# Luca96/carla-driving-rl-agent

Hardware: AMD Instinct MI355X
Metric: PPO update-steps/sec (batch=256, 4x90x120x3 obs) (higher is better)
Workload: dtype f32; 1 GPU; configs[1]: synthetic rollout buffer 256x4-frame 90x120x3 obs per GPU, full CARLANetwork fwd/bwd + PPO (re-sampled Beta, pathwise) / value loss + clip + Adam, fp32; per_gpu_batch=256, global_batch=256, parallelism=dp1, policy_loss=resampled (reference-faithful)

## Files before the change

### carla-driving-rl-agent_amd/_lib.py

```python
import ctypes as C
import os

_HERE = os.path.dirname(os.path.abspath(__file__))
LIB_PATH = os.path.join(_HERE, 'libcdrl_hip.so')


class CdrlError(RuntimeError):
    pass


class Config(C.Structure):
    _fields_ = [('B', C.c_int32), ('T', C.c_int32), ('H', C.c_int32), ('W', C.c_int32),
                ('road', C.c_int32), ('vehicle', C.c_int32), ('navigation', C.c_int32), ('A', C.c_int32),
                ('stem', C.c_int32), ('stage_c', C.c_int32 * 3), ('stage_n', C.c_int32 * 3), ('last', C.c_int32),
                ('feat', C.c_int32), ('rnn_image', C.c_int32), ('rnn_small', C.c_int32), ('dyn', C.c_int32),
                ('head', C.c_int32), ('exp_scale', C.c_float), ('compute', C.c_int32),
                ('freeze_trunk', C.c_int32), ('optimizer', C.c_int32), ('polyak', C.c_float), ('train_stats', C.c_int32),
                ('clip_mode', C.c_int32), ('skip_nonfinite', C.c_int32)]


class TrainStatsLayout(C.Structure):
    _fields_ = [(n, C.c_int32) for n in ('rows', 'width', 'header', 'kind', 't_head', 't_dynamics', 'lr', 'lr_dynamics', 'clip_ratio',
                                         'entropy_coef', 'speed', 'similarity', 'metrics', 'norms', 'trunk_norms', 'n_policy',
                                         'n_value', 'n_trunk')]
# ... 54 lines not shown

_i, _i64, _f, _d, _sz = C.c_int, C.c_int64, C.c_float, C.c_double, C.c_size_t
_L = C.c_void_p
_V = C.POINTER(View)
_pp = C.POINTER(C.c_void_p)

PROTOTYPES = {
    'cdrl_last_error': (C.c_char_p, []),
    'cdrl_version': (_i, []),
    'cdrl_env_overrides': (_i, [C.c_char_p, _i]),
    'cdrl_diag_active': (_i, []),
    'cdrl_crc32c': (C.c_uint32, [C.c_uint32, C.c_void_p, C.c_size_t]),
    'cdrl_config_default': (None, [C.POINTER(Config)]),
    'cdrl_optimizer_slots': (_i, [_i, C.POINTER(C.c_int32), C.POINTER(C.c_float)]),
    'cdrl_learner_create': (_i, [C.POINTER(Config), C.POINTER(_L)]),
    'cdrl_learner_destroy': (None, [_L]),
    'cdrl_learner_param_count': (_i, [_L, _i]),
    'cdrl_learner_param_info': (_i, [_L, _i, _i, C.POINTER(ParamInfo)]),
    'cdrl_learner_region_offset': (_i64, [_L, _i, _i]),
    'cdrl_learner_region_elems': (_i64, [_L, _i, _i]),
    'cdrl_learner_params_total': (_i64, [_L]),
    'cdrl_learner_grads_total': (_i64, [_L]),
    'cdrl_learner_workspace_bytes': (_sz, [_L]),
    'cdrl_learner_bind': (_i, [_L, _fp, _fp, _fp, _fp, _fp, _sz]),
    'cdrl_learner_set_hparams': (_i, [_L, C.POINTER(HParams), _fp]),
    'cdrl_learner_share_hparams': (_i, [_L, _L]),
    'cdrl_learner_set_comm_stream': (_i, [_L, _fp]),
    'cdrl_learner_tail_offset': (_i64, [_L]),
    'cdrl_learner_reset_optimizer_steps': (_i, [_L, _fp]),
    'cdrl_learner_get_optimizer_state': (_i, [_L, C.POINTER(OptimizerState), _fp]),
    'cdrl_learner_set_optimizer_state': (_i, [_L, C.POINTER(OptimizerState), _fp]),
    'cdrl_learner_gate_stats': (_i, [_L, C.POINTER(GateStats), _fp]),
    'cdrl_learner_gate_reset': (_i, [_L, _fp]),
    'cdrl_learner_train_stats_layout': (_i, [_L, C.POINTER(TrainStatsLayout)]),
    'cdrl_learner_train_stats_buffer': (_i, [_L, C.POINTER(C.c_void_p), C.POINTER(_i64)]),
    'cdrl_learner_train_stats_reset': (_i, [_L, _fp]),
    'cdrl_learner_policy_forward_backward': (_i, [_L, C.POINTER(PolicyBatch), _f, _fp]),
    'cdrl_learner_policy_forward': (_i, [_L, _fp, _fp, _fp, _fp, _fp]),
    'cdrl_learner_policy_backward': (_i, [_L, C.POINTER(PolicyBatch), _f, _fp]),
    'cdrl_learner_policy_forward_backward_resample': (_i, [_L, C.POINTER(PolicyBatch), C.c_uint64, C.c_uint64, _f, _fp]),
    'cdrl_pwconv_x3_packed_bytes': (_i64, [_i]),
    'cdrl_pwconv_x3_packed_bytes_n': (_i64, [_i, _i]),
    'cdrl_pwconv_x3_partial_rows': (_i, [_i, _i, _i, _i]),
    'cdrl_pwconv_x3_pack': (_i, [_fp, _i, _i, _i, _i, _fp, _fp]),
    'cdrl_pwconv_x3': (_i, [_fp, _i, _i, _fp, _fp, _fp, _fp, _i, _i, _i, _i, _i, _i, _fp, _fp]),
    'cdrl_pwconv_x3_wide_bwd_rows': (_i, [_i]),
    'cdrl_pwconv_x3_wide_bwd': (_i, [_fp, _i, _i, _i, _i, _fp, _fp, _fp, _fp, _fp, _i, _i, _i, _i, _i, _i, _i, _fp, _fp, _fp, _fp, _fp]),
    'cdrl_pwconv_bwd_fused_workspace': (_i64, [_i, _i, _i, _i, _i]),
    'cdrl_pwconv_bwd_fused': (_i, [_fp, _i, _i, _i, _i, _fp, _fp, _fp, _fp, _i, _i, _fp, _fp, _fp, _fp, _fp, _fp, _fp, C.c_void_p, _fp, _i,
                                   _i, _i, _fp, _fp, _fp, C.c_void_p, _i, _i, _i, _i, C.c_void_p]),
    'cdrl_gemm_x3_packed_bytes': (_i64, [_i, _i]),
    'cdrl_gemm_x3_pack': (_i, [_fp, _i, _i, _i, _i, _fp, _fp]),
    'cdrl_gemm_x3': (_i, [_fp, _i, _i, _fp, _fp, _fp, _i, _i, _i, _i, _i, _i, _fp]),
    'cdrl_f32_to_bf16': (_i, [_fp, _fp, _i64, _fp]),
    'cdrl_bf16_to_f32': (_i, [_fp, _fp, _i64, _fp]),
    'cdrl_pwconv_bf16_partial_rows': (_i, [_i, _i, _i, _i]),
    'cdrl_pwconv_bf16_packed_elems': (_i64, [_i]),
    'cdrl_pwconv_bf16_pack': (_i, [_fp, _i, _i, _fp, _fp]),
    'cdrl_pwconv_bf16': (_i, [_fp, _i, _i, _fp, _fp, _fp, _fp, _fp, _i, _i, _i, _i, _i, _i, _fp, _fp]),
    'cdrl_gru_step_fwd': (_i, [_fp] * 9 + [_i, _i, _fp]),
    'cdrl_gru_step_bwd': (_i, [_fp, _i] + [_fp] * 9 + [_i, _i, _fp]),
    'cdrl_beta_sample_logp': (_i, [_fp, _fp, _i, _i, _i, C.c_uint64, C.c_uint64, _fp, _fp, _fp]),
    'cdrl_beta_sample': (_i, [_fp, _fp, _i, _i, _i, C.c_uint64, C.c_uint64, _fp, _fp, _fp, _fp]),
    'cdrl_beta_act': (_i, [_fp, _fp, _i, _i, _i, C.c_uint64, C.c_uint64, _fp, _fp, _fp, _fp, _fp]),
    'cdrl_gamma_implicit_grad': (_i, [_fp, _fp, _i, _fp, _fp]),
    'cdrl_beta_sample_gammas': (_i, [_fp, _fp, _i, _i, _i, C.c_uint64, C.c_uint64, _fp, _fp]),
    'cdrl_philox_words': (_i, [C.c_uint64, C.c_uint64, C.c_uint64, _i, _i, _fp, _fp]),
    'cdrl_learner_policy_apply': (_i, [_L, _fp]),
    'cdrl_learner_joint_forward_backward': (_i, [_L, C.POINTER(PolicyBatch), _fp, _f, _fp]),
    'cdrl_learner_joint_forward_backward_resample': (_i, [_L, C.POINTER(PolicyBatch), _fp, C.c_uint64, C.c_uint64, _f, _fp]),
    'cdrl_learner_joint_apply': (_i, [_L, _fp]),
    'cdrl_learner_clone_forward_backward': (_i, [_L, C.POINTER(CloneBatch), _f, _f, _f, _f, _fp]),
    'cdrl_learner_repr_forward_backward': (_i, [_L, _fp, _fp, _fp, _fp, _f, _f, _fp]),
    'cdrl_learner_trunk_apply': (_i, [_L, _fp]),
    'cdrl_learner_sequence_begin': (_i, [_L, _fp]),
    'cdrl_learner_sequence_end': (_i, [_L, _fp]),
    'cdrl_learner_value_forward_backward': (_i, [_L, C.POINTER(ValueBatch), _f, _fp]),
    'cdrl_learner_value_apply': (_i, [_L, _fp]),
    'cdrl_learner_update_old_policy': (_i, [_L, _fp]),
    'cdrl_learner_predict': (_i, [_L, _fp, _fp, _fp, _fp, _fp, _fp, _fp, _fp]),
    'cdrl_learner_trunk_forward_train': (_i, [_L, _fp, _fp, _fp, _fp, _fp]),
    'cdrl_learner_get_buffer': (_i, [_L, _i, C.POINTER(_fp), C.POINTER(_i64)]),
    'cdrl_learner_named_buffer': (_i, [_L, C.c_char_p, C.POINTER(C.c_void_p), C.POINTER(_i64)]),
    'cdrl_learner_check_guards': (_i, [_L, _fp, C.POINTER(_i64), C.POINTER(_i64)]),
    'cdrl_gae_returns': (_i, [_fp, _fp, _i, _d, _d, _f, _fp, _fp, _fp, _fp, _fp, _fp]),
    'cdrl_gae_returns_segments': (_i, [_fp, _fp, _fp, _i, _i, _d, _d, _f, _fp, _fp, _fp, _fp, _fp, _fp]),
    'cdrl_gae_segments_scratch_doubles': (_i64, [_i, _i]),
    'cdrl_gather_rows': (_i, [_fp, _fp, _fp, _i, _i64, _fp]),
    'cdrl_gemm_nn': (_i, [_fp, _i, _i, _fp, _i, _i, _fp, _fp, _i, _i, _i, _i, _i, _i, _fp]),
    'cdrl_gemm_tn_workspace_elems': (_i64, [_i, _i, _i]),
    'cdrl_gemm_tn': (_i, [_fp, _i, _i, _fp, _i, _i, _fp, _i, _i, _i, _fp, _i, _fp]),
    'cdrl_bn_small_fwd': (_i, [_fp, _i, _i, _fp, _fp, _fp, _fp, _fp, _fp, _fp]),
    'cdrl_bn_small_bwd': (_i, [_fp, _fp, _i, _i, _fp, _fp, _fp, _fp, _fp, _fp]),
    'cdrl_bn_small_bwd_pair': (_i, [_fp, _fp, _fp, _i, _i] + [_fp] * 10),
    'cdrl_linear_heads_fwd': (_i, [_fp, _i, _fp, _fp, _fp, _fp, _i, _i, _fp]),
    'cdrl_linear_heads_bwd': (_i, [_fp, _i, _fp, _fp, _fp, _fp, _fp, _fp, _i, _i, _fp]),
    'cdrl_stem_fwd': (_i, [_fp, _fp, _fp, _fp, _i, _i, _i, _i, _i, _fp]),
    'cdrl_stem_fwd_stats_rows': (_i, [_i] * 5),
    'cdrl_stem_fwd_stats': (_i, [_fp] * 5 + [_i] * 5 + [_fp]),
    'cdrl_stem_bwd_workspace_doubles': (_i64, [_i, _i, _i, _i, _i]),
    'cdrl_stem_bwd_filter': (_i, [_fp, _fp, _fp, _fp, _i, _i, _i, _i, _i, _fp, _fp]),
    'cdrl_dwconv_fwd': (_i, [_fp, _fp, _fp, _fp, _i, _i, _i, _i, _i, _fp]),
    'cdrl_dwconv_bwd_data': (_i, [_fp, _fp, _fp, _i, _i, _i, _i, _i, _fp]),
    'cdrl_dwconv_bwd_workspace_doubles': (_i64, [_i, _i, _i, _i, _i]),
    'cdrl_dwconv_bwd_filter': (_i, [_fp, _fp, _fp, _fp, _i, _i, _i, _i, _i, _fp, _fp]),
    'cdrl_augment_workspace_floats': (_i64, [_i, _i, _i]),
# ... 122 lines not shown
```

### carla-driving-rl-agent_amd/csrc/capi.hip

```cpp
#include <stdlib.h>
#include <string.h>

#include <new>

#include "../../include/cdrl.h"
#include "engine.h"

using namespace cdrl;

struct cdrl_learner {
    Learner* impl;
};

static inline hipStream_t S(void* s) { return reinterpret_cast<hipStream_t>(s); }

#define CHECK_L(l)                         \
    if (!(l) || !(l)->impl) {              \
        cdrl::set_error("null learner");   \
        return -1;                         \
    }

static inline bool bad_act_type(int at) {
    if (at == 0 || at == 1) return false;
    cdrl::set_error("act_type: 0 (float32) or 1 (bf16)");
// ... 718 lines not shown
    }
    PwBwdFused f;
    f.dz = make_view(const_cast<float*>(dz), ld_dz, dz_coff);
    f.dz_shuffle = dz_shuffle;
    f.act = act;
    f.y = y;
    f.stats = stats;
    f.coef = coef;
    f.a = make_view(const_cast<float*>(a), lda, a_coff);
    f.a_stats = a_stats;
    f.a_gamma = a_gamma;
    f.a_beta = a_beta;
    f.a_dgamma = a_dgamma;
    f.a_dbeta = a_dbeta;
    f.a_coef = a_coef;
    f.W = W;
    f.Wp = W_packed;
    f.da = make_view(da, ldda, da_coff);
    f.accumulate = accumulate;
    f.dW = dW;
    f.db = db;
    f.qpart = qpart;
    f.dbpart = dbpart;
    f.G = G;
    f.Mg = Mg;
    f.N = N;
    f.K = K;
    f.at = act_type;
    CDRL_TRY(pw_bwd_fused(f, S(stream)));
    return pw_bwd_fused_reduce(f, S(stream));
}

int64_t cdrl_gemm_x3_packed_bytes(int N, int K) { return gemm_x3_packed_bytes(N, K); }

int cdrl_gemm_x3_pack(const float* B, int K, int N, int sbk, int sbn, void* packed, void* stream) {
    if (!B || !packed) return -1;
    GemmX3Pack e = gemm_x3_pack_entry(B, packed, K, N, sbk, sbn);
    GemmX3Pack* d = nullptr;
    if (hipMalloc(reinterpret_cast<void**>(&d), sizeof(e)) != hipSuccess) return -2;
    int rc = hipMemcpy(d, &e, sizeof(e), hipMemcpyHostToDevice) == hipSuccess ? gemm_x3_pack_many(d, 1, S(stream)) : -2;
    (void)hipStreamSynchronize(S(stream));
    (void)hipFree(d);
    return rc;
}

int cdrl_gemm_x3(const float* A, int lda, int a_coff, const void* B_packed, const float* bias, float* C, int ldc, int c_coff, int M,
                 int N, int K, int accumulate, int act_type, void* stream) {
    if (!A || !B_packed || !C) {
        cdrl::set_error("cdrl_gemm_x3: null argument");
        return -1;
    }
    return gemm_x3(make_view(const_cast<float*>(A), lda, a_coff), B_packed, bias, make_view(C, ldc, c_coff), M, N, K, accumulate,
                   S(stream), act_type != 0, act_type);
}

int cdrl_f32_to_bf16(const float* x, void* y, int64_t n, void* stream) {
    if (!x || !y) return -1;
    return f32_to_bf16(x, y, n, S(stream));
}

int cdrl_bf16_to_f32(const void* x, float* y, int64_t n, void* stream) {
    if (!x || !y) return -1;
    return bf16_to_f32(x, y, n, S(stream));
}

int cdrl_pwconv_bf16_partial_rows(int G, int Mg, int N, int K) { return pw_bf16_partial_rows(G, Mg, N, K); }

int64_t cdrl_pwconv_bf16_packed_elems(int K) { return pw_bf16_packed_elems(K); }

int cdrl_pwconv_bf16_pack(const float* W, int K, int N, void* packed, void* stream) {
    if (!W || !packed) return -1;
    return pw_bf16_pack(W, K, N, packed, S(stream));
}

int cdrl_pwconv_bf16(const void* A, int lda, int a_coff, const float* pro_stats, const float* W, const void* W_packed,
                     const float* bias, void* C, int ldc, int c_coff, int G, int Mg, int N, int K, double* part, void* stream) {
    if (!A || (!W && !W_packed) || !C) {
        cdrl::set_error("cdrl_pwconv_bf16: null argument");
        return -1;
    }
    return pw_bf16(A, lda, a_coff, pro_stats, W, bias, C, ldc, c_coff, G, Mg, N, K, part, S(stream), W_packed);
}

int cdrl_gru_step_fwd(const float* xp, const float* hprev, const float* R, const float* b1, float* z, float* r, float* hh,
                      float* hp, float* hnew, int B, int u, void* stream) {
    if (!xp || !hprev || !R || !b1 || !z || !r || !hh || !hp || !hnew) {
        cdrl::set_error("cdrl_gru_step_fwd: null argument");
        return -1;
    }
    return gru_step_fwd(xp, hprev, R, b1, z, r, hh, hp, hnew, View{nullptr, 0, 0}, B, u, S(stream));
}

int cdrl_gru_step_bwd(const float* dh, int ld_dh, const float* z, const float* r, const float* hh, const float* hp,
                      const float* hprev, const float* RT, float* dxp, float* dhp, float* dhprev, int B, int u, void* stream) {
    if (!dh || !z || !r || !hh || !hp || !hprev || !RT || !dxp || !dhp) {
        cdrl::set_error("cdrl_gru_step_bwd: null argument");
        return -1;
    }
    return gru_step_bwd(make_view(const_cast<float*>(dh), ld_dh), z, r, hh, hp, hprev, RT, dxp, dhp, dhprev, B, u, S(stream));
}

int cdrl_gather_rows(const float* src, const int32_t* idx, float* dst, int nrows, int64_t row_elems, void* stream) {
    if (!src || !idx || !dst) {
        cdrl::set_error("cdrl_gather_rows: null argument");
        return -1;
    }
// ... 735 lines not shown
```

### carla-driving-rl-agent_amd/csrc/cdrl_kernels.h

```cpp
#pragma once
#include "cdrl_common.h"

namespace cdrl {

int colstats(View y, int G, int Mg, int C, double* part, hipStream_t st, int at = 0);
int bn_finalize(const double* part, int nb, int G, int Mg, int C, const float* gamma, const float* beta,
                float* mov_mean, float* mov_var, int bessel, int training, float* stats ,
                hipStream_t st);
struct BnInfEntry {
    const float *gamma, *beta, *mov_mean, *mov_var;
    float* stats;
    int G, C;
};
int bn_inference_stats_many(const BnInfEntry* tab_dev, int n, int max_c, hipStream_t st);
int bn_apply(View y, int G, int Mg, int C, const float* stats, int act, View dst, int shuffle_ctot,
             hipStream_t st, const View* pass_src = nullptr, const View* pass_dst = nullptr, int at = 0);
int bn_small_fwd(View x, int M, int C, const float* gamma, const float* beta, float* mov_mean, float* mov_var, float* stats,
                 View out, hipStream_t st);
int bn_small_bwd(View dout, View x, int M, int C, const float* stats, float* dgamma, float* dbeta, float* coef, float* dx,
                 hipStream_t st);
int bn_small_bwd_pair(View doutA, View doutB, View x, int M, int C, const float* statsA, const float* statsB, float* dgammaA,
                      float* dbetaA, float* coefA, float* dgammaB, float* dbetaB, float* coefB, float* dx, hipStream_t st);
struct PoolSrc {
    const uint8_t* argmax;
// ... 244 lines not shown
    float* db = nullptr;
    float* qpart = nullptr;
    double* dbpart = nullptr;
    int N = 0, K = 0, G = 1, Mg = 0;
    int at = 0;
    const double* fin_part = nullptr;
    double* fin_tot = nullptr;
    int fin_nb = 0;
    float* o_dgamma = nullptr;
    float* o_dbeta = nullptr;
};
enum PwbRefusal {
    PWB_OK = 0,
    PWB_REFUSE_SHAPE = 1,
    PWB_REFUSE_ALIGN = 2,
    PWB_REFUSE_PADDING = 3,
    PWB_REFUSE_2GB = 4,
    PWB_REFUSE_GROUPS = 5,
    PWB_REFUSE_FIN = 6,
    PWB_REFUSE_ANORM = 7,
};
struct PwbPlan {
    int ok, refusal;
    int form;
    int kp, np, bm;
    int tiles, nbpg;
    int wp_ks;
    int shuf, anorm, acc, fin;
    int coef_needed;
    int lds_bytes;
    int64_t qpart_elems, dbpart_elems;
    int64_t spart_offset;
    char why[192];
};
PwbPlan pw_bwd_fused_plan(const PwBwdFused& f);
bool pw_bwd_fused_supported(View dz, View a, View da, int N, int K, int at = 0);
int pw_bwd_fused_nbpg(int G, int Mg, int N, int K, int at = 0);
int64_t pw_bwd_fused_qpart_elems(int G, int Mg, int N, int K, int at = 0);
int64_t pw_bwd_fused_dbpart_elems(int G, int Mg, int N, int K, int at = 0);
int pw_bwd_fused(const PwBwdFused& f, hipStream_t st);
int pw_bwd_fused_reduce(const PwBwdFused& f, hipStream_t st);

struct GemmX3Pack {
    const float* w;
    __bf16* wp;
    int K, N, sbk, sbn, KS, NP;
};
bool gemm_x3_supported(View A, int K);
int64_t gemm_x3_packed_bytes(int N, int K);
GemmX3Pack gemm_x3_pack_entry(const float* w, void* wp, int K, int N, int sbk, int sbn);
int gemm_x3_pack_many(const GemmX3Pack* tab_dev, int n, hipStream_t st);
int pack_all(const GemmX3Pack* tg, int ng, const PwPack* tp, int np, const PwX3Pack* t3, int n3, const PwTranspose* tt, int nt,
             int transpose_tiles, hipStream_t st);
int gemm_x3(View A, const void* Bp, const float* bias, View C, int M, int N, int K, int accumulate, hipStream_t st,
            bool bf16_operands = false, int at = 0);

bool pw_bf16_supported(int lda, int a_coff, int N, int K);
int pw_bf16_partial_rows(int G, int Mg, int N, int K);
int pw_bf16(const void* A, int lda, int a_coff, const float* pro_stats, const float* W, const float* bias, void* C, int ldc,
            int c_coff, int G, int Mg, int N, int K, double* part, hipStream_t st, const void* Wp = nullptr);
int64_t pw_bf16_packed_elems(int K);
int pw_bf16_pack(const float* W, int K, int N, void* Wp, hipStream_t st);
int f32_to_bf16(const float* x, void* y, int64_t n, hipStream_t st);
int bf16_to_f32(const void* x, float* y, int64_t n, hipStream_t st);

#define HEADS_MAX 4
#define HEADS_MAX_OUT 8
struct HeadSet {
    int nheads;
    int n[HEADS_MAX], off[HEADS_MAX];
    const float* w[HEADS_MAX];
    const float* b[HEADS_MAX];
    float* gw[HEADS_MAX];
    float* gb[HEADS_MAX];
};
int heads_fwd(const float* a, int lda, const HeadSet& hs, float* lin, int ldl, int B, int K, hipStream_t st);
int heads_bwd(const float* a, int lda, const HeadSet& hs, const float* dlin, int ldl, float* da, int ldda, int B, int K,
              hipStream_t st);

bool gru_step_supported(int u);
int gru_step_fwd(const float* xp, const float* hprev, const float* R, const float* b1, float* z, float* r, float* hh, float* hp,
                 float* hnew, View out, int B, int u, hipStream_t st);
int gru_step_bwd(View dh, const float* z, const float* r, const float* hh, const float* hp, const float* hprev, const float* RT,
                 float* dxp, float* dhp, float* dhprev, int B, int u, hipStream_t st);

struct PolicyLossArgs {
    const float* lin;
    const float* adv;
    const float* old_logp;
    const float* speed;
    const float* similarity;
    const float* u;
    const float* du_da;
    const float* du_db;
    const float* hp;
    float* dlin;
    float* metrics;
    float* aux;
    int B, A;
    float inv_world;
};
int policy_loss(const PolicyLossArgs& a, hipStream_t st);
struct CloneLossArgs {
    const float* lin;
    const float* u;
    const float* weight;
    const float* speed;
    const float* similarity;
// ... 143 lines not shown
```

### carla-driving-rl-agent_amd/csrc/gemm_x3.hip

```cpp
#include "colreduce.h"
#include "pack_bodies.h"

namespace cdrl {

typedef float f32x16 __attribute__((ext_vector_type(16)));
typedef __bf16 bf16x8 __attribute__((ext_vector_type(8)));
typedef __bf16 bf16x4 __attribute__((ext_vector_type(4)));

struct GemmX3Args {
    View A;
    const __bf16* Bp;
    const float* bias;
    View C;
    int accumulate;
    int M, N, K, KS, NP;
};

__device__ __forceinline__ void gx3_split(float x, __bf16& h1, __bf16& h2, __bf16& h3) {
    h1 = (__bf16)x;
    const float r1 = x - (float)h1;
    h2 = (__bf16)r1;
    h3 = (__bf16)(r1 - (float)h2);
}

// ... 89 lines not shown
                    c = __builtin_amdgcn_mfma_f32_32x32x16_bf16(af[0][i], bf[2][j], c, 0, 0, 0);
                    c = __builtin_amdgcn_mfma_f32_32x32x16_bf16(af[1][i], bf[1][j], c, 0, 0, 0);
                    c = __builtin_amdgcn_mfma_f32_32x32x16_bf16(af[1][i], bf[0][j], c, 0, 0, 0);
                    c = __builtin_amdgcn_mfma_f32_32x32x16_bf16(af[0][i], bf[1][j], c, 0, 0, 0);
                }
                c = __builtin_amdgcn_mfma_f32_32x32x16_bf16(af[0][i], bf[0][j], c, 0, 0, 0);
                acc[i][j] = c;
            }
    };
    bf16x8 b0[NS][2], b1[NS][2];
    u32x4_t raA[4], raB[4];
    load_stage(0, raA);
    load_b(0, b0);
    if (nstage > 1) load_stage(1, raB);
    store_stage(0, raA);
    if (nstage > 2) load_stage(2, raA);
    __syncthreads();
    auto iter = [&](int s, u32x4_t (&ruse)[4]) {
        const int buf = s & 1, ks = 2 * s;
        if (ks + 1 < a.KS) load_b(ks + 1, b1);
        mma(buf, 0, b0);
        if (ks + 1 < a.KS) {
            if (ks + 2 < a.KS) load_b(ks + 2, b0);
            mma(buf, 1, b1);
        }
        if (s + 1 < nstage) store_stage(buf ^ 1, ruse);
        if (s + 3 < nstage) load_stage(s + 3, ruse);
        __syncthreads();
    };
    for (int s = 0; s < nstage; s += 2) {
        iter(s, raB);
        if (s + 1 < nstage) iter(s + 1, raA);
    }
#pragma unroll
    for (int j = 0; j < 2; ++j) {
        const int n = n0 + wc * 64 + j * 32 + lrow;
        if (n >= N) continue;
        const float bv = a.bias ? a.bias[n] : 0.0f;
#pragma unroll
        for (int i = 0; i < 2; ++i)
#pragma unroll
            for (int r = 0; r < 16; ++r) {
                const int64_t m = m0 + wr * 64 + i * 32 + (r & 3) + 8 * (r >> 2) + 4 * lk;
                if (m < a.M) {
                    T* c = vptr<T>(a.C) + m * a.C.ld + a.C.coff + n;
                    float v = acc[i][j][r] + bv;
                    if (a.accumulate) v += ldf(c);
                    stf(c, v);
                }
            }
    }
}

__global__ void gemm_x3_pack_kernel(const GemmX3Pack* __restrict__ tab) {
    const GemmX3Pack d = tab[blockIdx.y];
    gemm_x3_pack_body(d, blockIdx.x, gridDim.x);
}

int64_t gemm_x3_packed_bytes(int N, int K) { return (int64_t)3 * cdiv(K, 16) * 2 * (cdiv(N, 128) * 128) * 8 * 2; }

GemmX3Pack gemm_x3_pack_entry(const float* w, void* wp, int K, int N, int sbk, int sbn) {
    GemmX3Pack e;
    e.w = w;
    e.wp = reinterpret_cast<__bf16*>(wp);
    e.K = K;
    e.N = N;
    e.sbk = sbk;
    e.sbn = sbn;
    e.KS = cdiv(K, 16);
    e.NP = cdiv(N, 128) * 128;
    return e;
}

int gemm_x3_pack_many(const GemmX3Pack* tab_dev, int n, hipStream_t st) {
    if (n <= 0) return 0;
    hipLaunchKernelGGL(gemm_x3_pack_kernel, dim3(32, n), dim3(256), 0, st, tab_dev);
    CDRL_LAUNCH_CHECK();
    return 0;
}

bool gemm_x3_supported(View A, int K) {
    return K >= 4 && K % 4 == 0 && A.ld % 4 == 0 && A.coff % 4 == 0 && (reinterpret_cast<uintptr_t>(A.p) & 15) == 0;
}

int gemm_x3(View A, const void* Bp, const float* bias, View C, int M, int N, int K, int accumulate, hipStream_t st, bool bf16_operands,
            int at) {
    if (M <= 0 || N <= 0) return 0;
    if (!gemm_x3_supported(A, K) || !Bp) {
        set_error("gemm_x3: unsupported alignment K=%d ld=%d coff=%d", K, A.ld, A.coff);
        return -1;
    }
    if ((int64_t)M * A.ld * 4 >= (int64_t)1 << 31) {
        set_error("gemm_x3: operand of 2 GB or more");
        return -1;
    }
    GemmX3Args a{A, reinterpret_cast<const __bf16*>(Bp), bias, C, accumulate, M, N, K, cdiv(K, 16), cdiv(N, 128) * 128};
    if (at && !bf16_operands) {
        set_error("gemm_x3: bf16 activation storage needs the bf16-operand variant");
        return -1;
    }
    if (at) hipLaunchKernelGGL((gemm_x3_kernel<1, true>), dim3(cdiv(M, 128), cdiv(N, 128)), dim3(256), 0, st, a);
    else if (bf16_operands) hipLaunchKernelGGL(gemm_x3_kernel<1>, dim3(cdiv(M, 128), cdiv(N, 128)), dim3(256), 0, st, a);
    else hipLaunchKernelGGL(gemm_x3_kernel<3>, dim3(cdiv(M, 128), cdiv(N, 128)), dim3(256), 0, st, a);
    CDRL_LAUNCH_CHECK();
    return 0;
}

}
```

### include/cdrl.h

```cpp
#ifndef CDRL_H
#define CDRL_H

#include <stddef.h>
#include <stdint.h>

#ifdef __cplusplus
extern "C" {
#endif

#define CDRL_VERSION 1

typedef struct cdrl_learner cdrl_learner;

typedef struct cdrl_config {
    int32_t B, T, H, W;
    int32_t road, vehicle, navigation, A;
    int32_t stem;
    int32_t stage_c[3];
    int32_t stage_n[3];
    int32_t last;
    int32_t feat, rnn_image, rnn_small, dyn, head;
    float exp_scale;
    int32_t compute;
    int32_t freeze_trunk;
// ... 142 lines not shown
    CDRL_BUF_AUX_V = 5,
    CDRL_BUF_LIN_P = 6,
    CDRL_BUF_LIN_V = 7,
    CDRL_BUF_SAMPLE = 8,
    CDRL_BUF_METRICS_R = 9
};
int cdrl_learner_get_buffer(const cdrl_learner* l, int which, float** ptr, int64_t* elems);
int cdrl_learner_named_buffer(const cdrl_learner* l, const char* name, void** ptr, int64_t* bytes);
int cdrl_learner_check_guards(cdrl_learner* l, void* stream, int64_t* bad_bands, int64_t* first_bad_offset);

int cdrl_gae_returns(const float* rewards, const float* values_be, int N, double gamma, double lambda, float scale,
                     float* returns, float* returns_be, float* adv_raw, float* adv, double* scratch, void* stream);
int cdrl_gae_returns_segments(const float* rewards, const float* values_be, const int32_t* seg_off, int S, int N,
                              double gamma, double lambda, float scale,
                              float* returns, float* returns_be, float* adv_raw, float* adv,
                              double* scratch, void* stream);
int64_t cdrl_gae_segments_scratch_doubles(int N, int S);

int cdrl_beta_sample(const float* alpha, const float* beta, int rows, int A, int ld, uint64_t seed, uint64_t offset,
                     float* u, float* du_dalpha, float* du_dbeta, void* stream);
int cdrl_beta_sample_logp(const float* alpha, const float* beta, int rows, int A, int ld, uint64_t seed, uint64_t offset,
                          float* u, float* log_prob, void* stream);
#define CDRL_ACT_STATS(A) (3 * (A) + 2)
int cdrl_beta_act(const float* dist, const float* value, int rows, int A, int mode, uint64_t seed, uint64_t offset,
                  const int32_t* active, float* action, float* log_prob, double* stats, void* stream);
int cdrl_gamma_implicit_grad(const double* a, const double* g, int n, double* out, void* stream);
int cdrl_beta_sample_gammas(const float* alpha, const float* beta, int rows, int A, int ld, uint64_t seed, uint64_t offset,
                            double* gammas, void* stream);
int cdrl_philox_words(uint64_t seed, uint64_t offset, uint64_t idx0, int n, int nblocks, uint32_t* out, void* stream);

int64_t cdrl_pwconv_x3_packed_bytes(int K);
int64_t cdrl_pwconv_x3_packed_bytes_n(int K, int N);
int cdrl_pwconv_x3_partial_rows(int G, int Mg, int N, int K);
int cdrl_pwconv_x3_pack(const float* W, int K, int N, int sbk, int sbn, void* packed, void* stream);
int cdrl_pwconv_x3(const float* A, int lda, int a_coff, const float* pro_stats, const void* W_packed, const float* bias, float* C,
                   int ldc, int c_coff, int G, int Mg, int N, int K, double* part, void* stream);
int cdrl_pwconv_x3_wide_bwd_rows(int Mg);
int cdrl_pwconv_x3_wide_bwd(const float* dz, int ld_dz, int dz_coff, int dz_shuffle, int act, const float* y, const float* stats,
                            const float* coef, const void* W_packed, float* da, int ldda, int da_coff, int accumulate, int G, int Mg,
                            int Cin, int Cout, double* part2, const float* ey, const float* epi_stats, double* part, void* stream);


int64_t cdrl_pwconv_bwd_fused_workspace(int G, int Mg, int N, int K, int which, int act_type);
int cdrl_pwconv_bwd_fused(const float* dz, int ld_dz, int dz_coff, int dz_shuffle, int act, const float* y, const float* stats,
                          const float* coef, const float* a, int lda, int a_coff, const float* a_stats, const float* a_gamma,
                          const float* a_beta, float* a_dgamma, float* a_dbeta, float* a_coef, const float* W, const void* W_packed,
                          float* da, int ldda, int da_coff, int accumulate, float* dW, float* db, float* qpart, double* dbpart, int G,
                          int Mg, int N, int K, int act_type, void* stream);

int64_t cdrl_gemm_x3_packed_bytes(int N, int K);
int cdrl_gemm_x3_pack(const float* B, int K, int N, int sbk, int sbn, void* packed, void* stream);
int cdrl_gemm_x3(const float* A, int lda, int a_coff, const void* B_packed, const float* bias, float* C, int ldc, int c_coff, int M,
                 int N, int K, int accumulate, int act_type, void* stream);

int cdrl_f32_to_bf16(const float* x, void* y, int64_t n, void* stream);
int cdrl_bf16_to_f32(const void* x, float* y, int64_t n, void* stream);
int cdrl_pwconv_bf16_partial_rows(int G, int Mg, int N, int K);
int64_t cdrl_pwconv_bf16_packed_elems(int K);
int cdrl_pwconv_bf16_pack(const float* W, int K, int N, void* packed, void* stream);
int cdrl_pwconv_bf16(const void* A, int lda, int a_coff, const float* pro_stats, const float* W, const void* W_packed,
                     const float* bias, void* C, int ldc, int c_coff, int G, int Mg, int N, int K, double* part, void* stream);

int cdrl_gru_step_fwd(const float* xp, const float* hprev, const float* R, const float* b1, float* z, float* r, float* hh,
                      float* hp, float* hnew, int B, int u, void* stream);
int cdrl_gru_step_bwd(const float* dh, int ld_dh, const float* z, const float* r, const float* hh, const float* hp,
                      const float* hprev, const float* RT, float* dxp, float* dhp, float* dhprev, int B, int u, void* stream);

int cdrl_gather_rows(const float* src, const int32_t* idx, float* dst, int nrows, int64_t row_elems, void* stream);

int cdrl_gemm_nn(const float* A, int lda, int a_coff, const float* B, int sbk, int sbn, const float* bias, float* C,
                 int ldc, int c_coff, int M, int N, int K, int accumulate, void* stream);
int64_t cdrl_gemm_tn_workspace_elems(int M, int N, int K);
int cdrl_gemm_tn(const float* A, int lda, int a_coff, const float* D, int ldd, int d_coff, float* out, int M, int N,
                 int K, float* workspace, int accumulate, int act_type, void* stream);
int cdrl_stem_fwd(const float* x, const float* w, const float* bias, float* y, int B, int T, int H, int W, int Cout,
                  void* stream);
int cdrl_stem_fwd_stats_rows(int B, int T, int H, int W, int Cout);
int cdrl_stem_fwd_stats(const float* x, const float* w, const float* bias, float* y, double* part, int B, int T, int H, int W, int Cout,
                        int act_type, void* stream);
int64_t cdrl_stem_bwd_workspace_doubles(int B, int T, int H, int W, int Cout);
int cdrl_stem_bwd_filter(const float* x, const float* dy, float* dw, float* db, int B, int T, int H, int W, int Cout,
                         double* workspace, void* stream);
int cdrl_dwconv_fwd(const float* a, const float* w, const float* bias, float* y, int N, int H, int W, int C, int stride,
                    void* stream);
int cdrl_dwconv_bwd_data(const float* dy, const float* w, float* da, int N, int H, int W, int C, int stride, void* stream);
int64_t cdrl_dwconv_bwd_workspace_doubles(int N, int H, int W, int C, int stride);
int cdrl_dwconv_bwd_filter(const float* a, const float* dy, float* dw, float* db, int N, int H, int W, int C, int stride,
                           double* workspace, void* stream);
int cdrl_pwconv_fused_partial_rows(int G, int Mg, int N, int K);
int cdrl_pwconv_fused(const float* a, int lda, int a_coff, const float* pro_stats, const float* w, int sbk, int sbn,
                      const float* bias, float* c, int ldc, int c_coff, int accumulate, int G, int Mg, int N, int K,
                      int epilogue, const float* epi_y, const float* epi_stats, double* part, void* stream);
int64_t cdrl_pwconv_pack_elems(int N, int K);
int cdrl_pwconv_pack(const float* W, int K, int N, int sbk, int sbn, float* packed, int bf16, void* stream);
int cdrl_pwconv_fused_packed(const float* a, int lda, int a_coff, const float* pro_stats, const float* w, int sbk, int sbn,
                             const float* bias, float* c, int ldc, int c_coff, int accumulate, int G, int Mg, int N, int K,
                             int epilogue, const float* epi_y, const float* epi_stats, double* part, const float* w_packed,
                             int packed_bf16, int act_type, void* stream);
int64_t cdrl_pwconv_bn_bwd_workspace_bytes(int G, int Mg, int N, int K);
int cdrl_pwconv_bn_bwd(const float* dout, int dout_ld, int dout_coff, int shuffle_ctot, int relu6, const float* y,
                       const float* stats, const float* x, int x_ld, int x_coff, const float* x_pro_stats, const float* w,
                       int G, int Mg, int N, int K, float* dgamma, float* dbeta, float* coef, float* dx, int dx_ld,
                       int dx_coff, int accumulate, float* dw, float* db, void* workspace, int act_type, void* stream);
int cdrl_pwconv_bn_bwd_packed(const float* dout, int dout_ld, int dout_coff, int shuffle_ctot, int relu6, const float* y,
                              const float* stats, const float* x, int x_ld, int x_coff, const float* x_pro_stats, const float* w,
                              int G, int Mg, int N, int K, float* dgamma, float* dbeta, float* coef, float* dx, int dx_ld,
// ... 120 lines not shown
```

Before: 80.59 update-steps/s.

## Add software-pipelined 96-row fp32 split-bf16 GEMM kernel with planner

Adds a new fp32 three-plane (split-bf16 x3) GEMM kernel that uses 96-row tiles and double-buffered LDS. Global loads of A and B and the bf16 split/store of A are interleaved with the MFMA chains under explicit scheduling barriers. A planner makes this form the default for fp32 operands with M >= 96 and exposes plan and explicit-form entry points. The goal is to hide memory latency and give more workgroups on mid-size M, at the cost of register pressure from prefetched B fragments and a more complex tail path.

```diff
diff --git a/carla-driving-rl-agent_amd/_lib.py b/carla-driving-rl-agent_amd/_lib.py
--- a/carla-driving-rl-agent_amd/_lib.py
+++ b/carla-driving-rl-agent_amd/_lib.py
@@ -130,6 +130,8 @@
     'cdrl_gemm_x3_packed_bytes': (_i64, [_i, _i]),
     'cdrl_gemm_x3_pack': (_i, [_fp, _i, _i, _i, _i, _fp, _fp]),
     'cdrl_gemm_x3': (_i, [_fp, _i, _i, _fp, _fp, _fp, _i, _i, _i, _i, _i, _i, _fp]),
+    'cdrl_gemm_x3_plan': (_i, [_i] * 5 + [C.POINTER(C.c_int32), _i]),
+    'cdrl_gemm_x3_ex': (_i, [_fp, _i, _i, _fp, _fp, _fp, _i, _i, _i, _i, _i, _i, _i, _i, _fp]),
     'cdrl_f32_to_bf16': (_i, [_fp, _fp, _i64, _fp]),
     'cdrl_bf16_to_f32': (_i, [_fp, _fp, _i64, _fp]),
     'cdrl_pwconv_bf16_partial_rows': (_i, [_i, _i, _i, _i]),
diff --git a/carla-driving-rl-agent_amd/csrc/capi.hip b/carla-driving-rl-agent_amd/csrc/capi.hip
--- a/carla-driving-rl-agent_amd/csrc/capi.hip
+++ b/carla-driving-rl-agent_amd/csrc/capi.hip
@@ -794,6 +794,37 @@
     }
     return gemm_x3(make_view(const_cast<float*>(A), lda, a_coff), B_packed, bias, make_view(C, ldc, c_coff), M, N, K, accumulate,
                    S(stream), act_type != 0, act_type);
+}
+
+int cdrl_gemm_x3_plan(int M, int N, int K, int bf16_operands, int act_type, int32_t* fields, int n_out) {
+    if (bad_act_type(act_type)) return -1;
+    if (!fields && n_out > 0) {
+        cdrl::set_error("cdrl_gemm_x3_plan: no field array");
+        return -1;
+    }
+    if (M < 1 || N < 1 || K < 1 || (act_type && !bf16_operands)) {
+        cdrl::set_error("cdrl_gemm_x3_plan: empty product, or bf16 activation storage without bf16 operands");
+        return -1;
+    }
+    const GemmX3Plan p = gemm_x3_plan(M, N, K, bf16_operands != 0, act_type);
+    const int32_t v[] = {p.form, p.tile_m, p.tile_n, p.waves, p.gx, p.gy, p.lds_bytes, p.wg_per_cu};
+    int n = 0;
+    for (int32_t x : v) {
+        if (n < n_out) fields[n] = x;
+        ++n;
+    }
+    return n;
+}
+
+int cdrl_gemm_x3_ex(const float* A, int lda, int a_coff, const void* B_packed, const float* bias, float* C, int ldc, int c_coff, int M,
+                    int N, int K, int accumulate, int act_type, int form, void* stream) {
+    if (bad_act_type(act_type)) return -1;
+    if (!A || !B_packed || !C) {
+        cdrl::set_error("cdrl_gemm_x3_ex: null argument");
+        return -1;
+    }
+    return gemm_x3(make_view(const_cast<float*>(A), lda, a_coff), B_packed, bias, make_view(C, ldc, c_coff), M, N, K, accumulate,
+                   S(stream), act_type != 0, act_type, form);
 }
 
 int cdrl_f32_to_bf16(const float* x, void* y, int64_t n, void* stream) {
diff --git a/carla-driving-rl-agent_amd/csrc/cdrl_kernels.h b/carla-driving-rl-agent_amd/csrc/cdrl_kernels.h
--- a/carla-driving-rl-agent_amd/csrc/cdrl_kernels.h
+++ b/carla-driving-rl-agent_amd/csrc/cdrl_kernels.h
@@ -320,8 +320,16 @@
 int gemm_x3_pack_many(const GemmX3Pack* tab_dev, int n, hipStream_t st);
 int pack_all(const GemmX3Pack* tg, int ng, const PwPack* tp, int np, const PwX3Pack* t3, int n3, const PwTranspose* tt, int nt,
              int transpose_tiles, hipStream_t st);
+enum { GEMM_X3_GENERAL = 1, GEMM_X3_PIPELINED = 2, GEMM_X3_PIPE_ROWS = 96 };
+struct GemmX3Plan {
+    int form;
+    int tile_m, tile_n, waves;
+    int gx, gy;
+    int lds_bytes, wg_per_cu;
+};
+GemmX3Plan gemm_x3_plan(int M, int N, int K, bool bf16_operands, int at, int form = 0);
 int gemm_x3(View A, const void* Bp, const float* bias, View C, int M, int N, int K, int accumulate, hipStream_t st,
-            bool bf16_operands = false, int at = 0);
+            bool bf16_operands = false, int at = 0, int form = 0);
 
 bool pw_bf16_supported(int lda, int a_coff, int N, int K);
 int pw_bf16_partial_rows(int G, int Mg, int N, int K);
diff --git a/carla-driving-rl-agent_amd/csrc/gemm_x3.hip b/carla-driving-rl-agent_amd/csrc/gemm_x3.hip
--- a/carla-driving-rl-agent_amd/csrc/gemm_x3.hip
+++ b/carla-driving-rl-agent_amd/csrc/gemm_x3.hip
@@ -165,6 +165,155 @@
     }
 }
 
+__device__ __forceinline__ void gx3_block(f32x16& acc, const bf16x8& a0, const bf16x8& a1, const bf16x8& a2, const bf16x8& b0, const bf16x8& b1,
+                                          const bf16x8& b2) {
+    f32x16 c = acc;
+    c = __builtin_amdgcn_mfma_f32_32x32x16_bf16(a2, b0, c, 0, 0, 0);
+    c = __builtin_amdgcn_mfma_f32_32x32x16_bf16(a0, b2, c, 0, 0, 0);
+    c = __builtin_amdgcn_mfma_f32_32x32x16_bf16(a1, b1, c, 0, 0, 0);
+    c = __builtin_amdgcn_mfma_f32_32x32x16_bf16(a1, b0, c, 0, 0, 0);
+    c = __builtin_amdgcn_mfma_f32_32x32x16_bf16(a0, b1, c, 0, 0, 0);
+    c = __builtin_amdgcn_mfma_f32_32x32x16_bf16(a0, b0, c, 0, 0, 0);
+    acc = c;
+}
+
+__global__ void __launch_bounds__(256, 2) gemm_x3_pipe_kernel(GemmX3Args a) {
+    constexpr int RT = GEMM_X3_PIPE_ROWS / 32;
+    constexpr int BM = 32 * RT, BK = 32, LDA = BK + 8;
+    constexpr int PLANE = BM * LDA, BUF = 3 * PLANE;
+    __shared__ __attribute__((aligned(16))) __bf16 As[2 * BUF];
+    const int tid = threadIdx.x, lane = tid & 63, wave = tid >> 6;
+    const int lrow = lane & 31, lk = lane >> 5;
+    const int64_t m0 = (int64_t)blockIdx.x * BM;
+    const int n0 = blockIdx.y * 128;
+    const int K = a.K, N = a.N, KS = a.KS;
+    const int nfull = KS >> 1;
+    typedef uint32_t u32x4_t __attribute__((ext_vector_type(4)));
+    const uint32_t OOR = 0x80000000u;
+    const __amdgpu_buffer_rsrc_t rsA = __builtin_amdgcn_make_buffer_rsrc(a.A.p, 0, (int)((int64_t)a.M * a.A.ld * 4), 0x00020000);
+    const uint32_t planeB = (uint32_t)KS * 2u * (uint32_t)a.NP * 16u;
+    const __amdgpu_buffer_rsrc_t rsB = __builtin_amdgcn_make_buffer_rsrc(const_cast<__bf16*>(a.Bp), 0, (int)(3u * planeB), 0x00020000);
+    const int cr = tid >> 3, ck = 4 * (tid & 7);
+    uint32_t aoff[RT];
+#pragma unroll
+    for (int i = 0; i < RT; ++i) {
+        const int64_t m = m0 + cr + 32 * i;
+        aoff[i] = m < a.M ? (uint32_t)((m * a.A.ld + a.A.coff + ck) * 4) : OOR;
+    }
+    auto load_a = [&](int s, int i) __attribute__((always_inline)) -> u32x4_t {
+        const uint32_t off = s * BK + ck < K ? aoff[i] + (uint32_t)(s * BK * 4) : OOR;
+        return __builtin_amdgcn_raw_buffer_load_b128(rsA, off, 0, 0);
+    };
+    const int wofs = cr * LDA + ck;
+    auto split_store = [&](int buf, int i, u32x4_t r) __attribute__((always_inline)) {
+        bf16x4 h[3];
+#pragma unroll
+        for (int e = 0; e < 4; ++e) {
+            __bf16 h1, h2, h3;
+            gx3_split(__uint_as_float(r[e]), h1, h2, h3);
+            h[0][e] = h1;
+            h[1][e] = h2;
+            h[2][e] = h3;
+        }
+#pragma unroll
+        for (int p = 0; p < 3; ++p) *reinterpret_cast<bf16x4*>(&As[buf * BUF + p * PLANE + 32 * i * LDA + wofs]) = h[p];
+    };
+    const int rofs = lrow * LDA + 8 * lk;
+    bf16x8 af[3][RT];
+    auto read_a = [&](int buf, int kk, int i) __attribute__((always_inline)) {
+#pragma unroll
+        for (int p = 0; p < 3; ++p) af[p][i] = *reinterpret_cast<const bf16x8*>(&As[buf * BUF + p * PLANE + 32 * i * LDA + rofs + 16 * kk]);
+    };
+    const uint32_t vb = (uint32_t)(lk * a.NP + n0 + wave * 32 + lrow) * 16u;
+    auto load_b = [&](int ks, bf16x8 (&bf)[3]) __attribute__((always_inline)) {
+        const uint32_t v = ks < KS ? vb : OOR;
+        const uint32_t so = (uint32_t)ks * 2u * (uint32_t)a.NP * 16u;
+#pragma unroll
+        for (int p = 0; p < 3; ++p) bf[p] = __builtin_bit_cast(bf16x8, __builtin_amdgcn_raw_buffer_load_b128(rsB, v, so + p * planeB, 0));
+    };
+    f32x16 acc[RT];
+#pragma unroll
+    for (int i = 0; i < RT; ++i)
+#pragma unroll
+        for (int r = 0; r < 16; ++r) acc[i][r] = 0.0f;
+    bf16x8 bq[4][3];
+    u32x4_t ra[RT], r0[RT];
+#pragma unroll
+    for (int i = 0; i < RT; ++i) r0[i] = load_a(0, i);
+    load_b(0, bq[0]);
+    load_b(1, bq[1]);
+#pragma unroll
+    for (int i = 0; i < RT; ++i) ra[i] = load_a(1, i);
+    load_b(2, bq[2]);
+    load_b(3, bq[3]);
+    __builtin_amdgcn_sched_barrier(0);
+#pragma unroll
+    for (int i = 0; i < RT; ++i) split_store(0, i, r0[i]);
+    __syncthreads();
+#pragma unroll
+    for (int i = 0; i < RT; ++i) read_a(0, 0, i);
+    __builtin_amdgcn_sched_barrier(0);
+    auto kstep_tail = [&](bf16x8 (&bf)[3]) __attribute__((always_inline)) {
+#pragma unroll
+        for (int i = 0; i < RT; ++i) gx3_block(acc[i], af[0][i], af[1][i], af[2][i], bf[0], bf[1], bf[2]);
+    };
+    auto stage = [&](int s, int buf, bf16x8 (&bA)[3], bf16x8 (&bB)[3]) __attribute__((always_inline)) {
+#pragma unroll
+        for (int i = 0; i < RT; ++i) {
+            gx3_block(acc[i], af[0][i], af[1][i], af[2][i], bA[0], bA[1], bA[2]);
+            read_a(buf, 1, i);
+            split_store(buf ^ 1, i, ra[i]);
+            ra[i] = load_a(s + 2, i);
+            if (i == RT - 1) load_b(2 * s + 4, bA);
+#pragma unroll
+            for (int g = 0; g < 6; ++g) {
+                __builtin_amdgcn_sched_group_barrier(0x8, 1, 0);
+                __builtin_amdgcn_sched_group_barrier(0x2, 6, 0);
+            }
+            __builtin_amdgcn_sched_group_barrier(0x100, 3, 0);
+            __builtin_amdgcn_sched_group_barrier(0x200, 3, 0);
+            __builtin_amdgcn_sched_barrier(0);
+        }
+        __syncthreads();
+#pragma unroll
+        for (int i = 0; i < RT; ++i) {
+            gx3_block(acc[i], af[0][i], af[1][i], af[2][i], bB[0], bB[1], bB[2]);
+            read_a(buf ^ 1, 0, i);
+            if (i == RT - 1) load_b(2 * s + 5, bB);
+            __builtin_amdgcn_sched_group_barrier(0x8, 6, 0);
+            __builtin_amdgcn_sched_group_barrier(0x100, 3, 0);
+            __builtin_amdgcn_sched_barrier(0);
+        }
+    };
+    int s = 0;
+    for (; s + 1 < nfull; s += 2) {
+        stage(s, 0, bq[0], bq[1]);
+        stage(s + 1, 1, bq[2], bq[3]);
+    }
+    if (nfull & 1) {
+        stage(s, 0, bq[0], bq[1]);
+        if (KS & 1) kstep_tail(bq[2]);
+    } else if (KS & 1) {
+        kstep_tail(bq[0]);
+    }
+    const int n = n0 + wave * 32 + lrow;
+    if (n < N) {
+        const float bv = a.bias ? a.bias[n] : 0.0f;
+#pragma unroll
+        for (int i = 0; i < RT; ++i)
+#pragma unroll
+            for (int r = 0; r < 16; ++r) {
+                const int64_t m = m0 + i * 32 + (r & 3) + 8 * (r >> 2) + 4 * lk;
+                if (m < a.M) {
+                    float* c = vptr<float>(a.C) + m * a.C.ld + a.C.coff + n;
+                    float v = acc[i][r] + bv;
+                    if (a.accumulate) v += ldf(c);
+                    stf(c, v);
+                }
+            }
+    }
+}
+
 __global__ void gemm_x3_pack_kernel(const GemmX3Pack* __restrict__ tab) {
     const GemmX3Pack d = tab[blockIdx.y];
     gemm_x3_pack_body(d, blockIdx.x, gridDim.x);
@@ -196,8 +345,29 @@
     return K >= 4 && K % 4 == 0 && A.ld % 4 == 0 && A.coff % 4 == 0 && (reinterpret_cast<uintptr_t>(A.p) & 15) == 0;
 }
 
+GemmX3Plan gemm_x3_plan(int M, int N, int K, bool bf16_operands, int at, int form) {
+    GemmX3Plan p{};
+    p.form = form ? form : !bf16_operands && !at && M >= GEMM_X3_PIPE_ROWS ? GEMM_X3_PIPELINED : GEMM_X3_GENERAL;
+    p.tile_m = p.form == GEMM_X3_PIPELINED ? GEMM_X3_PIPE_ROWS : 128;
+    p.tile_n = 128;
+    p.waves = 4;
+    p.gx = cdiv(M, p.tile_m);
+    p.gy = cdiv(N, p.tile_n);
+    p.lds_bytes = 2 * (bf16_operands ? 1 : 3) * p.tile_m * (32 + 8) * 2;
+    p.wg_per_cu = 2;
+    return p;
+}
+
 int gemm_x3(View A, const void* Bp, const float* bias, View C, int M, int N, int K, int accumulate, hipStream_t st, bool bf16_operands,
-            int at) {
+            int at, int form) {
+    if (form < 0 || form > GEMM_X3_PIPELINED) {
+        set_error("gemm_x3: form %d (0 = planned, 1 = general, 2 = pipelined)", form);
+        return -1;
+    }
+    if (form == GEMM_X3_PIPELINED && (bf16_operands || at)) {
+        set_error("gemm_x3: the pipelined form is the float32 three-plane case only (bf16_operands=%d act_type=%d)", (int)bf16_operands, at);
+        return -1;
+    }
     if (M <= 0 || N <= 0) return 0;
     if (!gemm_x3_supported(A, K) || !Bp) {
         set_error("gemm_x3: unsupported alignment K=%d ld=%d coff=%d", K, A.ld, A.coff);
@@ -212,9 +382,12 @@
         set_error("gemm_x3: bf16 activation storage needs the bf16-operand variant");
         return -1;
     }
-    if (at) hipLaunchKernelGGL((gemm_x3_kernel<1, true>), dim3(cdiv(M, 128), cdiv(N, 128)), dim3(256), 0, st, a);
-    else if (bf16_operands) hipLaunchKernelGGL(gemm_x3_kernel<1>, dim3(cdiv(M, 128), cdiv(N, 128)), dim3(256), 0, st, a);
-    else hipLaunchKernelGGL(gemm_x3_kernel<3>, dim3(cdiv(M, 128), cdiv(N, 128)), dim3(256), 0, st, a);
+    const GemmX3Plan p = gemm_x3_plan(M, N, K, bf16_operands, at, form);
+    const dim3 grid(p.gx, p.gy), block(64 * p.waves);
+    if (at) hipLaunchKernelGGL((gemm_x3_kernel<1, true>), grid, block, 0, st, a);
+    else if (bf16_operands) hipLaunchKernelGGL(gemm_x3_kernel<1>, grid, block, 0, st, a);
+    else if (p.form == GEMM_X3_PIPELINED) hipLaunchKernelGGL(gemm_x3_pipe_kernel, grid, block, 0, st, a);
+    else hipLaunchKernelGGL(gemm_x3_kernel<3>, grid, block, 0, st, a);
     CDRL_LAUNCH_CHECK();
     return 0;
 }
diff --git a/include/cdrl.h b/include/cdrl.h
--- a/include/cdrl.h
+++ b/include/cdrl.h
@@ -218,6 +218,9 @@
 int cdrl_gemm_x3_pack(const float* B, int K, int N, int sbk, int sbn, void* packed, void* stream);
 int cdrl_gemm_x3(const float* A, int lda, int a_coff, const void* B_packed, const float* bias, float* C, int ldc, int c_coff, int M,
                  int N, int K, int accumulate, int act_type, void* stream);
+int cdrl_gemm_x3_plan(int M, int N, int K, int bf16_operands, int act_type, int32_t* fields, int n_out);
+int cdrl_gemm_x3_ex(const float* A, int lda, int a_coff, const void* B_packed, const float* bias, float* C, int ldc, int c_coff, int M,
+                    int N, int K, int accumulate, int act_type, int form, void* stream);
 
 int cdrl_f32_to_bf16(const float* x, void* y, int64_t n, void* stream);
 int cdrl_bf16_to_f32(const void* x, float* y, int64_t n, void* stream);
```

Result: no change. 80.84 update-steps/s (median of 4 runs) (+0.3%).
